# supabase/etl

Hardware: AMD Instinct MI355X
Metric: WAL bytes/s decoded (higher is better)
Workload: dtype u8; 1 GPU; cfg2_fixed_5xint4: 64 MiB batches of CopyData-framed pgoutput, device-resident in / device-resident out, offsets sidecar, NO_CONTROL | ASYNC; batch_bytes=67108819, frames_per_batch=594511, pool_batches=6, parallelism=shard1

## Files before the change

etl_amd/csrc/dev_types.h:

```cpp
#pragma once
#include <stdint.h>

namespace etlg {

enum : uint8_t { FT_BAD = 0 };

struct DevCol {
  uint8_t cls;
  uint8_t nullable;
  uint8_t identity;
  uint8_t key_col;
  uint16_t off_full;
  uint16_t off_key;
  uint16_t key_index;
  uint16_t hr;
};

struct DevSlot {
  uint32_t n_cols, n_ident;
  uint32_t row_full, row_key;
  uint32_t st_full, st_key;
  uint32_t cols_base;
  uint32_t has_var;
  uint32_t key_masks;
// ... 130 lines not shown
  uint32_t keys_base;
};

struct PlanParams {
  unsigned long long* desc;
  unsigned long long* d_clear;
  uint32_t clear_words;
  uint32_t ntiles;
  uint32_t lds_bytes;
  uint32_t rows_off;
  uint32_t n_tabs;
  const PlanTab* tabs;
  const uint32_t* cols;
  uint32_t dbg;
  uint32_t max_row_dw;
  const unsigned long long* pre;
  unsigned long long* pre_out;
  uint32_t* pre_ticket;
  uint32_t pre_tag;
  uint32_t pre_row_dw;
  uint32_t pre_key_dw;
  uint32_t pre_key_below;
  uint32_t pre_key_max;
};

struct ColSel {
  const uint8_t* ev_kind; const uint8_t* ev_flags; const uint32_t* ev_slot; const uint64_t* ev_body;
  uint64_t n_events;
  uint32_t slot, kinds;
  unsigned long long* host_rows;
  uint32_t row_full, row_key;
  uint32_t* blk;
  uint32_t nblocks;
  uint64_t* row_event; uint64_t* row_base;
  uint32_t pb, n_cols;
  uint32_t identity_pk;
  uint32_t pk_comparable;
  const uint8_t* fixed; const uint8_t* heap;
  const uint32_t* cols;
  const uint32_t* kcols;
  uint32_t dl, dl_ident;
  unsigned long long* ice;
};
constexpr unsigned long long kPbDelete = 1ull << 63, kPbKey = 1ull << 62, kPbSecond = 1ull << 61, kPbBase = (1ull << 61) - 1;

constexpr uint32_t kAkNumericStr = 64, kAkTimetzStr = 65, kAkJsonStr = 66;
// ... 74 lines not shown
```

etl_amd/csrc/host_orchestrate.inc:

```

namespace {

int32_t download_batch(etlg_ctx* c, etlg_batch* b) {
  OutSet* os = b->dev;
  if (!os) return ETLG_OK;
  if (!c->d2h_stream) HIPCHK(c, hipStreamCreateWithFlags(&c->d2h_stream, hipStreamNonBlocking));
  hipStream_t s = c->d2h_stream;
  etlg_batch_view& v = b->v;
  const size_t n = (size_t)v.n_events;
  const size_t o_start = 0, o_commit = o_start + al64(n * 8), o_ord = o_commit + al64(n * 8), o_body = o_ord + al64(n * 8);
  const size_t o_table = o_body + al64(n * 8), o_slot = o_table + al64(n * 4), o_kind = o_slot + al64(n * 4), o_flags = o_kind + al64(n);
  const size_t o_fixed = o_flags + al64(n), o_heap = o_fixed + al64((size_t)v.fixed_bytes), total = o_heap + al64((size_t)v.heap_bytes) + 64;
  if (b->h_arena_cap < total) {
    if (b->h_arena) { c->harena_pool.emplace_back(b->h_arena, b->h_arena_cap); b->h_arena = nullptr; b->h_arena_cap = 0; }
    size_t best = (size_t)-1;
    for (size_t i = 0; i < c->harena_pool.size(); i++)
      if (c->harena_pool[i].second >= total && (best == (size_t)-1 || c->harena_pool[i].second < c->harena_pool[best].second)) best = i;
    if (best != (size_t)-1) {
      b->h_arena = c->harena_pool[best].first; b->h_arena_cap = c->harena_pool[best].second;
      c->harena_pool.erase(c->harena_pool.begin() + (long)best);
    } else {
      const size_t cap = (total + (total >> 2) + 4095) & ~(size_t)4095;
      HIPCHK(c, hipHostMalloc((void**)&b->h_arena, cap, hipHostMallocDefault));
      b->h_arena_cap = cap;
// ... 314 lines not shown
  const uint64_t nf_avg = b->scan_chained && b->nf_est ? b->nf_est : nf;
  const uint64_t avg = (b->len + nf_avg - 1) / nf_avg;
  if (level == 0) {
    PlanParams& q = c->pq;
    q.ntiles = (nf + 63) / 64;
    uint64_t cap = 64 * avg * (100 + (uint64_t)c->plan_margin_pct) / 100 + 128;
    cap = std::min<uint64_t>((cap + 127) & ~127ull, 48 * 1024);
    q.rows_off = (uint32_t)std::max<uint64_t>(cap, 2048 + 64);
    q.lds_bytes = q.rows_off + (c->plan_max_row > 32 ? (uint32_t)(64ull * c->plan_max_row + 64) : 0u);
    q.n_tabs = c->n_plan_tabs; q.tabs = (const PlanTab*)((const uint8_t*)b->side->dev.p + b->side->o_ptabs); q.cols = (const uint32_t*)((const uint8_t*)b->side->dev.p + b->side->o_pcols);
    q.dbg = c->plan_dbg;
    q.max_row_dw = (c->plan_max_row + 3) / 4;
    const size_t gtiles = std::min<size_t>(64, (size_t)1 << etlg_k_plan_pre_group_log());
    const size_t per = 2 * ((size_t)q.ntiles + ((size_t)q.ntiles + gtiles - 1) / gtiles);
    const bool pre = c->plan_pre != 0 && c->plan_uniform_dw != 0;
    const size_t dbytes = per * 8 + 64;
    q.desc = nullptr; q.d_clear = nullptr; q.clear_words = 0;
    if (!pre) {
      uint8_t *dcur, *doth;
      RC(take_descriptors(c, dbytes, &dcur, &doth));
      q.desc = (unsigned long long*)dcur;
      q.d_clear = (unsigned long long*)doth; q.clear_words = (uint32_t)(dbytes / 8);
    }
    q.pre = nullptr; q.pre_out = nullptr; q.pre_ticket = nullptr; q.pre_tag = 0; q.pre_row_dw = c->plan_uniform_dw;
    q.pre_key_dw = c->plan_uniform_key_dw; q.pre_key_below = c->plan_deletes ? c->plan_key_below : 0u; q.pre_key_max = c->plan_deletes ? c->plan_key_max : 0u;
    if (pre) {
      constexpr uint32_t NB = etlg_ctx::kPreBufs;
      const size_t pbytes = (64 + per * 8 + 255) & ~(size_t)255;
      if (pbytes > c->pre_half) {
        HIPCHK(c, sync_decode_streams(c));
        const size_t half = (pbytes * 2 + 4095) & ~(size_t)4095;
        HIPCHK(c, c->d_pre.ensure(half * NB));
        HIPCHK(c, hipMemsetAsync(c->d_pre.p, 0, half * NB, c->stream));
        HIPCHK(c, hipStreamSynchronize(c->stream));
        c->pre_half = half;
      }
      const uint32_t useq = c->pre_seq++, slot = useq % NB;
      uint8_t* pbuf = (uint8_t*)c->d_pre.p + (size_t)slot * c->pre_half;
      q.pre_ticket = (uint32_t*)pbuf;
      q.pre_out = (unsigned long long*)(pbuf + 64);
      q.pre_tag = 1u + (useq / NB) % 3u;
      launch(c, kPlanPre, p);
      q.pre = q.pre_out;
      if (c->plan_pre == 1) q.dbg |= 512u;
    }
    launch(c, kPlan, p);
    b->used_fused = true; b->used_cells = false;
    return ETLG_OK;
  }
  FusedParams& q = c->fq;
  bool any_var = false;
  for (int32_t li : c->last_live) for (auto& sc : c->slots[(size_t)li]->cols) if (!fixed_class(sc.type_class)) any_var = true;
  int kernel = (avg <= 192 && !(any_var && cells_ok && avg > 96)) ? 0 : (cells_ok ? 2 : 1);
  if (c->fused_kernel >= 0 && c->fused_kernel <= 2) kernel = c->fused_kernel == 2 && !cells_ok ? 1 : c->fused_kernel;
  if (direct) kernel = 2;
  b->used_rows = false;
  if (kernel != 0 || c->fused_kernel == 4) {
    uint32_t maxh = 1, maxh_old = 0, maxrow = 16;
    bool ok = !b->copy.active && !(p.flags & kDecCopyRows) && !b->any_sync_done && !(c->fused_dbg & ~(8u | 32u)) && q.side_bytes != 0 && ((uintptr_t)p.in & 15) == 0 &&
              widest <= etlg_k_rows_max_cols() && !b->no_rows && c->rows_mode != 0 && (c->fused_kernel < 0 || c->fused_kernel == 4);
    for (int32_t li : c->last_live) {
      const SlotHost& sh = *c->slots[(size_t)li];
      uint32_t nh = 0, nhi = 0;
      for (auto& sc : sh.cols) if (!heapless_class(sc.type_class)) { nh++; if (sc.identity) nhi++; }
      maxh = std::max(maxh, nh); maxh_old = std::max(maxh_old, nhi);
      maxrow = std::max<uint32_t>(maxrow, sh.desc.row_bytes_full + std::max<uint32_t>(sh.desc.row_bytes_key, sh.desc.n_ident == sh.desc.n_cols ? sh.desc.row_bytes_full : 0u));
    }
// ... 531 lines not shown
```

etl_amd/csrc/host_state.h:

```cpp
#pragma once
#include <hip/hip_runtime_api.h>

#include <algorithm>
#include <cstddef>
#include <cstdio>
#include <cstdlib>
#include <cstring>
#include <chrono>
#include <map>
#include <mutex>
#include <memory>
#include <set>
#include <string>
#include <string_view>
#include <type_traits>
#include <unordered_map>
#include <vector>

#include "../../include/etlg.h"
#include "dev_types.h"

using namespace etlg;

extern "C" void etlg_k_launch(int which, const DecParams* p, hipStream_t s);
extern "C" const char* etlg_k_name(int which);
extern "C" void etlg_k_ctl_pick(const uint8_t* tags, uint32_t nframes, uint32_t* hdr, uint32_t* list, uint32_t cap, hipStream_t s);
extern "C" void etlg_k_shard_cuts(const uint8_t* tags, const uint32_t* offs, uint32_t nframes, uint32_t n_shards, uint32_t* cuts, hipStream_t s);
extern "C" void etlg_k_ctl_span(const uint8_t* tags, uint32_t nframes, const uint32_t* list, uint32_t n, uint32_t* span, hipStream_t s);
extern "C" void etlg_k_ctl_gather(const uint8_t* in, const uint32_t* offs, const uint32_t* frames, uint32_t nkeep, uint32_t* lens, const uint32_t* out_offs, uint8_t* out, hipStream_t s);
extern "C" void etlg_k_launch_fused(int blk, const DecParams* p, const void* q, hipStream_t s);
extern "C" int etlg_k_fused_set_lds(void);
extern "C" void etlg_k_launch_bounds(const uint8_t* in, uint64_t len, uint32_t* offs, uint32_t offs_cap, void* scratch, uint32_t* result, uint32_t* hints, uint32_t* hflag,
                                     int sequential, hipStream_t s);
extern "C" size_t etlg_k_bounds_scratch_bytes(size_t ntiles);
extern "C" uint32_t etlg_k_bounds_tile_bytes(void);
extern "C" uint32_t etlg_k_copy_bytes_per_row(uint32_t ncols);
extern "C" int etlg_k_copy_set_lds(void);
extern "C" void etlg_k_launch_copy(const uint8_t* rows, const uint32_t* row_offs, uint32_t nrows, uint64_t rows_len, uint32_t ncols,
                                   uint32_t rel_id, uint8_t* out, uint32_t* out_offs, uint32_t lds_bytes, int lane_per_byte, const DecParams* dec, hipStream_t s);
extern "C" void etlg_k_launch_cells(const DecParams* p, const void* q, hipStream_t s);
extern "C" void etlg_k_launch_plan(const DecParams* p, const void* q, hipStream_t s);
extern "C" void etlg_k_launch_plan_pre(const DecParams* p, const void* q, hipStream_t s);
extern "C" uint32_t etlg_k_plan_pre_group_log(void);
extern "C" int etlg_k_plan_set_lds(void);
extern "C" void etlg_k_col_select(const void* sel, hipStream_t s);
extern "C" void etlg_k_col_cdc(const void* job, hipStream_t s);
extern "C" void etlg_k_col_fixed(const void* job, hipStream_t s);
extern "C" uint32_t etlg_k_col_pack_max(void);
extern "C" void etlg_k_col_fixed_pack(const void* jobs, uint32_t n, hipStream_t s);
extern "C" void etlg_k_col_var_pack(const void* jobs, uint32_t n, unsigned long long* const* blk, int64_t* const* offs, unsigned long long* const* tot, int step, hipStream_t s);
extern "C" void etlg_k_scan_lens(const uint32_t* lens, uint64_t n, unsigned long long* blk, int64_t* offsets, hipStream_t s);
extern "C" void etlg_k_col_list(const void* job, unsigned long long* blk, int64_t* offsets, int step, hipStream_t s);
extern "C" void etlg_k_size_hints(const void* job, hipStream_t s);
extern "C" void etlg_k_rowbinary(const void* job, unsigned long long* blk, int64_t* offsets, unsigned long long* tot, int step, hipStream_t s);
extern "C" void etlg_k_col_var(const void* job, unsigned long long* blk, int64_t* offsets, int step, hipStream_t s);
extern "C" int etlg_k_cells_set_lds(void);
extern "C" uint32_t etlg_k_cells_table_bytes(uint32_t maxc);
extern "C" uint32_t etlg_k_copy_cells_table_bytes(uint32_t maxc);
extern "C" uint32_t etlg_k_copy_cells_lds(uint32_t maxc, uint32_t window);
extern "C" void etlg_k_launch_copy_cells(const DecParams* p, const void* q, hipStream_t s);
extern "C" uint32_t etlg_k_cells_maxc(void);
extern "C" void etlg_k_launch_rows(const DecParams* p, const void* q, hipStream_t s);
extern "C" void etlg_k_finish(const void* job, unsigned long long* blk, int64_t* offsets, int step, hipStream_t st);
extern "C" int etlg_k_rows_set_lds(void);
extern "C" int etlg_k_rows_waves(void);
extern "C" int etlg_k_rows_waves_per_simd(void);
// ... 205 lines not shown
  int users = 0;
  hipEvent_t ready = nullptr;
  uint32_t synced = 0;
};

}

struct etlg_ctx {
  int device = 0;
  uint64_t gen = 0;
  hipStream_t stream = nullptr;
  bool own_stream = false;
  int32_t worker = ETLG_WORKER_APPLY;
  uint32_t sync_table = 0;
  uint64_t bootstrap = 0;
  ControlState cs;
  std::map<uint32_t, TState> states;
  std::vector<std::unique_ptr<SlotHost>> slots;
  bool slots_dirty = true;
  bool in_txn = false; uint64_t final_lsn = 0, next_ord = 0;
  size_t desc_half = 0;
  static constexpr uint32_t kPreBufs = 4;
  DevBuf d_pre; size_t pre_half = 0; uint32_t pre_seq = 0;
  size_t desc_dirty[4] = {0, 0, 0, 0};
  uint32_t desc_cur = 0;
  hipStream_t stream2 = nullptr;
  hipEvent_t tail2 = nullptr;
  bool tail2_set = false;
  hipEvent_t fence_ev = nullptr;
  bool hdr_in_flight = false;
  int overlap_mode = 1;
  bool debug_invariants = false;
  bool prof_serial = false;
  unsigned long long overlapped = 0;
  static constexpr uint32_t kResRing = 32;
  uint64_t scan_last_nf = 0, scan_last_len = 0;
  bool scan_chain_mode = true;
  uint64_t scan_chained_n = 0, scan_chain_redone = 0;
  bool chain_spare = true;
  uint64_t chain_spared = 0;
  uint64_t chain_healed = 0;
  uint64_t ring_recleared = 0;
  uint32_t res_seq = 0;
  DevResult* h_init_ring = nullptr;
  DevResult* d_init_ring = nullptr;
  CopyJob copy;
// ... 172 lines not shown
```

etl_amd/csrc/plan.hip:

```cpp
#include "lookback.hip.h"

namespace etlg {

struct WinLds {
  const ETLG_LDS_AS u8* base;
  DEV uint32_t w(uint32_t aoff) const { return ETLG_LDS_LD32(base + aoff); }
};
struct WinGlb {
  const u8* base; uint32_t lim;
  DEV uint32_t w(uint32_t aoff) const {
    uint32_t v = 0;
    if (aoff + 4 <= lim) __builtin_memcpy(&v, base + aoff, 4);
    else for (uint32_t k = 0; aoff + k < lim; k++) v |= (uint32_t)base[aoff + k] << (8 * k);
    return v;
  }
};
template <class M> DEV uint32_t rd32(const M& m, uint32_t off) {
  const uint32_t a = off & ~3u, s = off & 3u;
  return __builtin_amdgcn_alignbyte(m.w(a + 4), m.w(a), s);
}
template <class M> DEV uint64_t rd64(const M& m, uint32_t off) {
  const uint32_t a = off & ~3u, s = off & 3u;
  const uint32_t w0 = m.w(a), w1 = m.w(a + 4), w2 = m.w(a + 8);
  return __builtin_amdgcn_alignbyte(w1, w0, s) | ((uint64_t)__builtin_amdgcn_alignbyte(w2, w1, s) << 32);
// ... 41 lines not shown
    const uint32_t d2 = dig4(pad_word(__builtin_amdgcn_alignbyte(w3, w2, s), k, 2), bad);
    mag = (uint64_t)d0 * 100000000ull + (d1 * 10000u + d2);
    uint64_t lim;
    if (cls == ETLG_TC_U32) lim = 0xFFFFFFFFull;
    else if (cls == ETLG_TC_I16) lim = neg ? 0x8000ull : 0x7FFFull;
    else lim = neg ? 0x80000000ull : 0x7FFFFFFFull;
    ok = (n != 0u) & (nd != 0u) & (n <= 12u) & (nd <= 11u) & (bad == 0u) & (mag <= lim) & ((cls != ETLG_TC_U32) | (neg ^ 1u));
  }
  return neg ? 0 - mag : mag;
}

DEV int plan_find(const PlanParams& q, uint32_t rel_u) {
  const ETLG_CONST_AS uint32_t* t = (const ETLG_CONST_AS uint32_t*)(uintptr_t)q.tabs;
  int lo = 0, hi = (int)q.n_tabs - 1;
  while (lo <= hi) {
    const int mid = (lo + hi) >> 1;
    const uint32_t v = t[mid * (int)(sizeof(PlanTab) / 4)];
    if (v == rel_u) return mid;
    if (v < rel_u) lo = mid + 1; else hi = mid - 1;
  }
  return -1;
}

#define WSTAMP(k) do { if ((q.dbg & 64u) && threadIdx.x == 0) ((unsigned long long*)p.heap)[(size_t)blockIdx.x * 8 + (k)] = wall_clock64(); } while (0)
#define PSTAMP(k) do { if ((q.dbg & 32u) && threadIdx.x == 0 && (blockIdx.x & 15u) == 3u) { const unsigned long long t_ = clock64(); atomicAdd(&p.res->dbg_t[k], t_ - tprev); tprev = t_; } } while (0)

constexpr uint32_t kPreBeginLen = kBodyOff + 20u, kPreCommitLen = kBodyOff + 25u;
constexpr int kPreTilesPerWave = 8, kPreWaves = 8;
constexpr uint32_t pre_log2(uint32_t v) { return v <= 1u ? 0u : 1u + pre_log2(v >> 1); }
constexpr uint32_t kPreGroupLog = pre_log2(kPreTilesPerWave * kPreWaves);
static_assert((1u << kPreGroupLog) == (uint32_t)(kPreTilesPerWave * kPreWaves), "a group of the pre-pass is a power of two of tiles");
static_assert(kPreTilesPerWave <= 32 && kPreWaves <= 8, "cand_m / short_m are 32-bit masks; at most two waves per SIMD");
constexpr uint32_t kPlanMaxPolls = 1u << 15;

struct PlanPre2 { unsigned long long a0 = 0, l0 = 0, a1 = 0, l1 = 0; bool valid = false; };
struct PlanFold { uint32_t fx, mk, l0, l1; };
DEV PlanFold fold_id() { return PlanFold{0u, 0u, 0u, 0u}; }
DEV PlanFold fold_f(const PlanFold& a, const PlanFold& b) {
  return PlanFold{a.fx + b.fx, a.mk > b.mk ? a.mk : b.mk, b.mk ? b.l0 : a.l0, b.mk ? b.l1 : a.l1};
}
DEV PlanFold fold_of(unsigned long long a, unsigned long long l) {
  return PlanFold{(uint32_t)a, (uint32_t)(a >> 32) & 0x3FFFFFFFu, (uint32_t)l, (uint32_t)(l >> 32) & 0x3FFFFFFFu};
}
DEV unsigned long long fold_agg(const PlanFold& v) { return ((unsigned long long)v.mk << 32) | v.fx; }
DEV unsigned long long fold_lsn(const PlanFold& v) { return ((unsigned long long)v.l1 << 32) | v.l0; }
DEV unsigned long long pair_state(unsigned long long a, unsigned long long l) { const unsigned long long st = a & ST_MASK; return st == (l & ST_MASK) ? st : 0ull; }
DEV PlanFold fold_scan(PlanFold v) {
#define ETLG_P3_DPP(ctrl, rmask) { PlanFold o_; \
    o_.fx = (uint32_t)__builtin_amdgcn_update_dpp(0, (int)v.fx, ctrl, rmask, 0xF, false); o_.mk = (uint32_t)__builtin_amdgcn_update_dpp(0, (int)v.mk, ctrl, rmask, 0xF, false); \
    o_.l0 = (uint32_t)__builtin_amdgcn_update_dpp(0, (int)v.l0, ctrl, rmask, 0xF, false); o_.l1 = (uint32_t)__builtin_amdgcn_update_dpp(0, (int)v.l1, ctrl, rmask, 0xF, false); \
    v = fold_f(o_, v); }
  ETLG_P3_DPP(0x111, 0xF) ETLG_P3_DPP(0x112, 0xF) ETLG_P3_DPP(0x114, 0xF) ETLG_P3_DPP(0x118, 0xF) ETLG_P3_DPP(0x142, 0xA) ETLG_P3_DPP(0x143, 0xC)
#undef ETLG_P3_DPP
  return v;
}
// ... 280 lines not shown
  if (keep) {
#pragma unroll
    for (int d = 0; d < RD; d++) L.row[d] = rimg[d];
  }
  L.agg = agg; L.tile_lsn = tile_lsn; L.ex = ex; L.ex_lsn = ex_lsn; L.tot_mark = tot_mark; L.tot_fx = tot_fx; L.early = early; L.done = false;
}

DEV void plan_late_carry(DecParams& p, uint32_t* failp) {
  if (!(p.flags & 16u) || !p.carry) return;
  for (uint32_t polls = 0;; polls++) {
    if (__hip_atomic_load(&p.carry->carry_ready, __ATOMIC_ACQUIRE, __HIP_MEMORY_SCOPE_AGENT)) break;
    if (polls > kPlanMaxPolls) { if (threadIdx.x == 0) atomicOr(failp, 1u); break; }
    __builtin_amdgcn_s_sleep(8);
  }
  p.in_txn = __hip_atomic_load(&p.carry->out_in_txn, __ATOMIC_RELAXED, __HIP_MEMORY_SCOPE_AGENT);
  p.final_lsn = __hip_atomic_load(&p.carry->out_final_lsn, __ATOMIC_RELAXED, __HIP_MEMORY_SCOPE_AGENT);
  p.next_ord = __hip_atomic_load(&p.carry->out_next_ord, __ATOMIC_RELAXED, __HIP_MEMORY_SCOPE_AGENT);
  p.flags &= ~16u;
}

struct PlanPreWords { unsigned long long g0 = 0, g1 = 0, t0 = 0, t1 = 0; };
DEV PlanPreWords plan_pre_load(const PlanParams& q, uint32_t tile) {
  PlanPreWords w;
  if (q.pre && tile < q.ntiles) {
    const ETLG_CONST_AS unsigned long long* dt = (const ETLG_CONST_AS unsigned long long*)(uintptr_t)(q.pre + 2 * (size_t)tile);
    const ETLG_CONST_AS unsigned long long* dg = (const ETLG_CONST_AS unsigned long long*)(uintptr_t)(q.pre + 2 * ((size_t)q.ntiles + (tile >> kPreGroupLog)));
    w.t0 = dt[0]; w.t1 = dt[1]; w.g0 = dg[0]; w.g1 = dg[1];
  }
  return w;
}

template <int RD>
DEV void plan_resolve(DecParams& p, const PlanParams& q, uint32_t tile, PlanLocal<RD>& L, unsigned long long& tprev, const PlanPre2& pre = PlanPre2(), const PlanPreWords& pw = PlanPreWords()) {
  if (L.done) return;
  const uint32_t lane = threadIdx.x;
  const uint32_t f = tile * 64u + lane;
  uint32_t* failp = &p.res->fused_fail;
  uint32_t bad = L.bad;
  const bool isI = (L.tagf >> 16) & 1u, isB = (L.tagf >> 17) & 1u, isC = (L.tagf >> 18) & 1u;
  const uint32_t pm = L.pm;
  const uint64_t b_lsn = L.b_lsn;
  uint64_t ex = L.ex, ex_lsn = L.ex_lsn;

  if (q.pre) {
    const PlanFold r = fold_f(fold_of(pw.g0, pw.g1), fold_of(pw.t0, pw.t1));
    ex = fold_agg(r); ex_lsn = fold_lsn(r);
  }
  else if (!L.early) plan_resolve2(q.desc, q.desc + 2 * (size_t)q.ntiles, tile, L.agg, L.tile_lsn, failp, pre, ex, ex_lsn);
  PSTAMP(7);
  uint32_t pre_mark = (uint32_t)(ex >> 32);
  if (pre_mark == 0) {
    plan_late_carry(p, failp);
    if (p.in_txn) { pre_mark = 1u; ex |= 1ull << 32; }
  }
  const uint64_t pre_lsn = (pre_mark & 1u) && (pre_mark >> 1) != 0 ? ex_lsn : p.final_lsn;
  PSTAMP(4);
  WSTAMP(4);

  const uint32_t last = pre_mark > pm ? pre_mark : pm;
  const bool in_txn = (last & 1u) != 0;
  const uint32_t fb1 = last >> 1;
  uint64_t final_lsn = 0;
  {
    const bool here = in_txn && fb1 != 0 && fb1 - 1 >= tile * 64u;
    const uint32_t src = here ? fb1 - 1 - tile * 64u : 0u;
    const uint32_t lo = (uint32_t)__shfl((int)(uint32_t)b_lsn, (int)src, 64), hi = (uint32_t)__shfl((int)(uint32_t)(b_lsn >> 32), (int)src, 64);
    if (in_txn) final_lsn = here ? (((uint64_t)hi << 32) | lo) : pre_lsn;
  }
// ... 69 lines not shown
    const uint32_t payu = wave_last(wave_scan_add(is_upd ? vbytes : 0u));
    if (lane == 0 && payu) atomicAdd(&p.res->pay_shard[tile & 31][1], (unsigned long long)payu);
  }
  if (__ballot(is_del && vbytes != 0)) {
    const uint32_t payd = wave_last(wave_scan_add(is_del ? vbytes : 0u));
    if (lane == 0 && payd) atomicAdd(&p.res->pay_shard[tile & 31][2], (unsigned long long)payd);
  }
  if ((any_bad || !cap_ok) && lane == 0) atomicOr(failp, 2u);
}

struct TileSpan { uint32_t nt, span0, span1, my_o; };
DEV TileSpan plan_span(const DecParams& p, uint32_t tile) {
  const uint32_t lane = threadIdx.x;
  TileSpan t;
  const uint32_t f0 = tile * 64u;
  t.nt = p.nframes - f0 < 64u ? p.nframes - f0 : 64u;
  const ETLG_CONST_AS uint32_t* offs_c = (const ETLG_CONST_AS uint32_t*)(uintptr_t)p.offs;
  t.span0 = offs_c[f0]; t.span1 = offs_c[f0 + t.nt];
  t.my_o = lane < t.nt ? p.offs[f0 + lane] : t.span1;
  return t;
}

template <int RD>
DEV void plan_stage_local(DecParams& p, const PlanParams& q, u8* smem, uint32_t tile, const TileSpan& ts, unsigned long long& tprev, PlanLocal<RD>& L, bool keep) {
  const uint32_t lane = threadIdx.x;
  L.done = true;
  const uint32_t nt = ts.nt, span0 = ts.span0, span1 = ts.span1, my_o = ts.my_o;
  PSTAMP(0);
  const uint32_t a0 = span0 & ~15u;
  const bool staged = span1 > span0 && span1 <= p.in_len && (uint64_t)(span1 - a0) + 64 <= q.rows_off && !(q.dbg & 1u);
  if (staged) {
    const uint32_t npieces = (span1 - a0 + 1023u) >> 10;
    for (uint32_t k = 0; k < npieces; k++) {
      const uint32_t c = a0 + (k << 10) + (lane << 4);
      if (c < span1 && (uint64_t)c + 16 <= p.in_len) ETLG_GLDS16(p.in + c, smem + (k << 10));
    }
    const uint32_t tail = a0 + (((uint32_t)p.in_len - a0) & ~15u);
    if (tail < span1 && (uint64_t)tail + 16 > p.in_len && tail + lane < p.in_len && lane < 16) smem[tail - a0 + lane] = p.in[tail + lane];
    ETLG_VMEM_WAIT();
    PSTAMP(1);
    WSTAMP(1);
    if (q.dbg & 2u) { if (smem[lane * 97u] == 0xEE && smem[lane * 13u + 5u] == 0xEF && my_o == 0xFFFFFFF1u) atomicOr(&p.res->fused_fail, 2u); return; }
    const WinLds m{(const ETLG_LDS_AS u8*)smem};
    plan_local(p, q, m, smem, true, a0, tile, nt, my_o, span0, span1, tprev, L, keep);
  } else {
    const WinGlb m{p.in, (uint32_t)p.in_len};
    plan_local(p, q, m, smem, false, 0u, tile, nt, my_o, span0, span1, tprev, L, keep);
  }
}

DEV bool plan_frames_from_device(DecParams& p, PlanParams& q) {
  if (!p.nframes_dev) return true;
  const ETLG_CONST_AS uint32_t* r = (const ETLG_CONST_AS uint32_t*)(uintptr_t)p.nframes_dev;
  const uint32_t nf = r[0], flags = r[1] | r[2];
  if (flags != 0 || nf == 0 || nf > p.nframes) {
    if (blockIdx.x == 0 && threadIdx.x == 0) {
      atomicOr(&p.res->fused_fail, 32u);
      __hip_atomic_store(&p.res->carry_ready, 1u, __ATOMIC_RELEASE, __HIP_MEMORY_SCOPE_AGENT);
    }
    return false;
  }
  p.nframes = nf;
  q.ntiles = (nf + 63u) >> 6;
  return true;
}

template <bool TWO, int RD>
DEV void plan_kernel(DecParams& p, const PlanParams& q_in, u8* smem) {
  PlanParams q = q_in;
  const uint32_t lane = threadIdx.x;
  unsigned long long tprev = (q.dbg & 32u) ? clock64() : 0ull;
  const uint32_t tile = blockIdx.x;
  WSTAMP(0);
  if (q.clear_words) {
    const uint32_t per = (q.clear_words + gridDim.x - 1) / gridDim.x;
    for (uint32_t i = lane; i < per; i += 64) { const uint32_t w = blockIdx.x * per + i; if (w < q.clear_words) q.d_clear[w] = 0; }
  }
  if (!(p.flags & 16u) && !load_carry(p)) return;
  if (!plan_frames_from_device(p, q)) return;
  const uint32_t t0 = TWO ? 2u * blockIdx.x : blockIdx.x;
  if (t0 >= q.ntiles) return;
  const TileSpan sa = plan_span(p, t0);
  const PlanPreWords pwa = plan_pre_load(q, t0), pwb = TWO ? plan_pre_load(q, t0 + 1u) : PlanPreWords();
  TileSpan sb = sa;
  if (TWO && t0 + 1u < q.ntiles) sb = plan_span(p, t0 + 1u);
  PlanLocal<RD> A;
  plan_stage_local(p, q, smem, t0, sa, tprev, A, TWO);
  if (TWO) {
    const uint32_t t1 = t0 + 1u;
    PlanLocal<RD> B;
    B.done = true;
    if (t1 < q.ntiles) {
      __threadfence_block();
      __syncthreads();
      plan_stage_local(p, q, smem, t1, sb, tprev, B, false);
    }
    PlanPre2 preA, preB;
    if (!A.done && !A.early && !q.pre) preA = plan_prefetch2(q.desc, q.desc + 2 * (size_t)q.ntiles, t0);
    if (!B.done && !B.early && !q.pre) preB = plan_prefetch2(q.desc, q.desc + 2 * (size_t)q.ntiles, t1);
    plan_resolve(p, q, t0, A, tprev, preA, pwa);
    plan_resolve(p, q, t1, B, tprev, preB, pwb);
    plan_store<true>(p, q, t0, A, tprev);
    plan_store<false>(p, q, t1, B, tprev);
  } else {
    plan_resolve(p, q, t0, A, tprev, PlanPre2(), pwa);
    plan_store<false>(p, q, t0, A, tprev);
  }
}

__global__ __launch_bounds__(kPreWaves * 64) void k_plan_pre(DecParams p, PlanParams q) {
  __shared__ unsigned long long s_wagg[kPreWaves][2];
  if (!plan_frames_from_device(p, q)) return;
  if (blockIdx.x >= ((q.ntiles + (1u << kPreGroupLog) - 1u) >> kPreGroupLog)) return;
  const uint32_t lane = threadIdx.x & 63u, wave = (uint32_t)__builtin_amdgcn_readfirstlane((int)(threadIdx.x >> 6)), g = blockIdx.x;
  const uint32_t t0 = (g << kPreGroupLog) + wave * (uint32_t)kPreTilesPerWave;
  uint32_t o[kPreTilesPerWave + 1];
#pragma unroll
  for (int i = 0; i <= kPreTilesPerWave; i++) {
    const uint64_t f = (uint64_t)(t0 + (uint32_t)i) * 64u + lane;
    o[i] = p.offs[f < p.nframes ? f : p.nframes];
  }
  uint32_t cand_m = 0;
  uint32_t short_m = 0;
  uint32_t tagv[kPreTilesPerWave];
  uint64_t lsnv[kPreTilesPerWave];
#pragma unroll
  for (int i = 0; i < kPreTilesPerWave; i++) {
    const uint64_t f = (uint64_t)(t0 + (uint32_t)i) * 64u + lane;
    const uint32_t o0 = o[i];
    const uint32_t nxt = (uint32_t)__builtin_amdgcn_readfirstlane((int)o[i + 1]);
    const uint32_t o1 = (uint32_t)__builtin_amdgcn_update_dpp((int)nxt, (int)o0, 0x130, 0xF, 0xF, false);
    const uint32_t flen = o1 - o0;
    const bool cand = f < p.nframes && o1 > o0 && o1 <= p.in_len && (flen == kPreBeginLen || flen == kPreCommitLen || (flen >= q.pre_key_below && flen <= q.pre_key_max));
    tagv[i] = 0; lsnv[i] = 0;
    if (cand) { cand_m |= 1u << i; tagv[i] = p.in[o0 + 30] | (flen << 8); lsnv[i] = ld_be64(p.in + o0 + 31); }
    if (flen < q.pre_key_below) short_m |= 1u << i;
  }
  PlanFold run = fold_id();
  PlanFold keep = fold_id();
#pragma unroll
  for (int i = 0; i < kPreTilesPerWave; i++) {
    const uint32_t tile = t0 + (uint32_t)i;
    const uint64_t f = (uint64_t)tile * 64u + lane;
    const bool live = f < p.nframes;
    const bool cand = (cand_m >> i) & 1u;
    const uint32_t tag = tagv[i] & 0xFFu, flen = tagv[i] >> 8;
    const uint64_t lsn = lsnv[i];
    const bool isB = cand && flen == kPreBeginLen && tag == 'B', isC = cand && flen == kPreCommitLen && tag == 'C';
    const bool isDel = ((short_m >> i) & 1u) || (cand && tag == 'D' && flen <= q.pre_key_max);
    const unsigned long long mB = __ballot(isB), mC = __ballot(isC), mD = __ballot(live && isDel && !isB && !isC);
    const uint64_t base = (uint64_t)tile * 64u;
    const uint32_t nlive = base >= p.nframes ? 0u : (p.nframes - base < 64u ? (uint32_t)(p.nframes - base) : 64u);
    const uint32_t nB = (uint32_t)__builtin_popcountll(mB), nC = (uint32_t)__builtin_popcountll(mC), nD = (uint32_t)__builtin_popcountll(mD);
    const uint32_t tot_fx = 2u * nB + 4u * nC + q.pre_key_dw * nD + q.pre_row_dw * (nlive - nB - nC - nD);
    const unsigned long long mBC = mB | mC;
    uint32_t tot_mark = 0;
    if (mBC) {
      const uint32_t h = 63u - (uint32_t)__builtin_clzll(mBC);
      tot_mark = ((((uint32_t)base + h) + 1u) << 1) | (uint32_t)((mB >> h) & 1ull);
    }
    uint64_t tile_lsn = 0;
    if (tot_mark & 1u) {
      const int src = (int)((tot_mark >> 1) - 1u - tile * 64u);
      tile_lsn = ((uint64_t)(uint32_t)__builtin_amdgcn_readlane((int)(uint32_t)(lsn >> 32), src) << 32) | (uint32_t)__builtin_amdgcn_readlane((int)(uint32_t)lsn, src);
      tile_lsn &= ~(3ull << 62);
    }
    if (lane == (uint32_t)i) keep = run;
    run = fold_f(run, PlanFold{tot_fx, tot_mark, (uint32_t)tile_lsn, (uint32_t)(tile_lsn >> 32)});
  }
  if (lane == 0) { s_wagg[wave][0] = fold_agg(run); s_wagg[wave][1] = fold_lsn(run); }
  __syncthreads();
  PlanFold before = fold_id();
  for (uint32_t w = 0; w < wave; w++) before = fold_f(before, fold_of(s_wagg[w][0], s_wagg[w][1]));
  if (lane < (uint32_t)kPreTilesPerWave && t0 + lane < q.ntiles) {
    const PlanFold r = fold_f(before, keep);
    unsigned long long* d = q.pre_out + 2 * (size_t)(t0 + lane);
    d[0] = fold_agg(r); d[1] = fold_lsn(r);
  }
  if (wave != (uint32_t)kPreWaves - 1u) return;
  const uint32_t ng = (q.ntiles + (1u << kPreGroupLog) - 1u) >> kPreGroupLog;
  unsigned long long* gd = q.pre_out + 2 * (size_t)q.ntiles;
  const unsigned long long tagbits = (unsigned long long)q.pre_tag << 62;
  uint32_t ticket = 0;
  if (lane == 0) {
    const PlanFold all = fold_f(before, run);
    ETLG_ST_PAIR(gd + 2 * (size_t)g, tagbits | fold_agg(all), tagbits | fold_lsn(all));
    ticket = atomicAdd(q.pre_ticket, 1u);
  }
  ticket = (uint32_t)__builtin_amdgcn_readfirstlane((int)ticket);
  if (ticket != ng - 1u) return;
  PlanFold carry = fold_id();
  unsigned long long na = 0, nl = 0;
// ... 1 lines not shown
  for (uint32_t base = 0; base < ng; base += 64u) {
    const uint32_t gi = base + lane;
    unsigned long long a = gi < ng ? na : tagbits, l = gi < ng ? nl : tagbits;
    if (gi + 64u < ng) ETLG_LD_PAIR(gd + 2 * (size_t)(gi + 64u), na, nl);
    bool have = pair_state(a, l) == tagbits;
    bool gave_up = false;
    for (uint32_t polls = 0;; polls++) {
      if (!have) { ETLG_LD_PAIR(gd + 2 * (size_t)gi, a, l); have = pair_state(a, l) == tagbits; }
      if (!__ballot(!have)) break;
      if (polls > kPlanMaxPolls) { if (lane == 0) atomicOr(&p.res->fused_fail, 1u); gave_up = true; break; }
      __builtin_amdgcn_s_sleep(2);
    }
    const PlanFold inc = fold_scan(gi < ng ? fold_of(a, l) : fold_id());
    PlanFold exc;
    exc.fx = (uint32_t)__builtin_amdgcn_update_dpp(0, (int)inc.fx, 0x138, 0xF, 0xF, false); exc.mk = (uint32_t)__builtin_amdgcn_update_dpp(0, (int)inc.mk, 0x138, 0xF, 0xF, false);
    exc.l0 = (uint32_t)__builtin_amdgcn_update_dpp(0, (int)inc.l0, 0x138, 0xF, 0xF, false); exc.l1 = (uint32_t)__builtin_amdgcn_update_dpp(0, (int)inc.l1, 0x138, 0xF, 0xF, false);
    const PlanFold r = fold_f(carry, exc);
    if (gi < ng && !gave_up) { gd[2 * (size_t)gi] = fold_agg(r); gd[2 * (size_t)gi + 1] = fold_lsn(r); }
    carry = fold_f(carry, fold_lane63(inc));
  }
  if (lane == 0) __hip_atomic_store(q.pre_ticket, 0u, __ATOMIC_RELAXED, __HIP_MEMORY_SCOPE_AGENT);
}

__global__ __launch_bounds__(64, ETLG_PLAN_MINWAVES) void k_plan(DecParams p, PlanParams q) {
  ETLG_DYNAMIC_LDS(smem);
  plan_kernel<false, 1>(p, q, smem);
}

template <int RD>
__global__ __launch_bounds__(64, ETLG_PLAN_MINWAVES) void k_plan2(DecParams p, PlanParams q) {
  ETLG_DYNAMIC_LDS(smem);
  plan_kernel<true, RD>(p, q, smem);
}

}

extern "C" {

using namespace etlg;

void etlg_k_launch_plan_pre(const DecParams* p, const void* qv, hipStream_t s) {
  const PlanParams* q = (const PlanParams*)qv;
  hipLaunchKernelGGL(k_plan_pre, dim3((q->ntiles + (1u << kPreGroupLog) - 1u) >> kPreGroupLog), dim3(kPreWaves * 64), 0, s, *p, *q);
}

void etlg_k_launch_plan(const DecParams* p, const void* qv, hipStream_t s) {
  const PlanParams* q = (const PlanParams*)qv;
  if (q->lds_bytes == q->rows_off && q->max_row_dw <= 8u && !(q->dbg & 512u)) {
    if (q->max_row_dw <= 6u) hipLaunchKernelGGL(k_plan2<6>, dim3((q->ntiles + 1) / 2), dim3(64), q->lds_bytes, s, *p, *q);
    else hipLaunchKernelGGL(k_plan2<8>, dim3((q->ntiles + 1) / 2), dim3(64), q->lds_bytes, s, *p, *q);
  } else hipLaunchKernelGGL(k_plan, dim3(q->ntiles), dim3(64), q->lds_bytes, s, *p, *q);
}

uint32_t etlg_k_plan_pre_group_log(void) { return kPreGroupLog; }

int etlg_k_plan_set_lds(void) {
  const int a = hipFuncSetAttribute((const void*)k_plan, hipFuncAttributeMaxDynamicSharedMemorySize, 64 * 1024) == hipSuccess ? 0 : 1;
  const int b = hipFuncSetAttribute((const void*)k_plan2<6>, hipFuncAttributeMaxDynamicSharedMemorySize, 64 * 1024) == hipSuccess ? 0 : 1;
  const int c = hipFuncSetAttribute((const void*)k_plan2<8>, hipFuncAttributeMaxDynamicSharedMemorySize, 64 * 1024) == hipSuccess ? 0 : 1;
  return a | b | c;
}

}
```

Baseline: 1859 GB/s.

## Fuse plan pre-pass into plan kernel as leading producer and scanner blocks

```diff
diff --git a/etl_amd/csrc/dev_types.h b/etl_amd/csrc/dev_types.h
--- a/etl_amd/csrc/dev_types.h
+++ b/etl_amd/csrc/dev_types.h
@@ -176,6 +176,7 @@
   uint32_t pre_key_dw;
   uint32_t pre_key_below;
   uint32_t pre_key_max;
+  uint32_t pre_fused;
 };
 
 struct ColSel {
diff --git a/etl_amd/csrc/host_orchestrate.inc b/etl_amd/csrc/host_orchestrate.inc
--- a/etl_amd/csrc/host_orchestrate.inc
+++ b/etl_amd/csrc/host_orchestrate.inc
@@ -360,11 +360,16 @@
       q.desc = (unsigned long long*)dcur;
       q.d_clear = (unsigned long long*)doth; q.clear_words = (uint32_t)(dbytes / 8);
     }
-    q.pre = nullptr; q.pre_out = nullptr; q.pre_ticket = nullptr; q.pre_tag = 0; q.pre_row_dw = c->plan_uniform_dw;
+    q.pre = nullptr; q.pre_out = nullptr; q.pre_ticket = nullptr; q.pre_tag = 0; q.pre_fused = 0; q.pre_row_dw = c->plan_uniform_dw;
     q.pre_key_dw = c->plan_uniform_key_dw; q.pre_key_below = c->plan_deletes ? c->plan_key_below : 0u; q.pre_key_max = c->plan_deletes ? c->plan_key_max : 0u;
     if (pre) {
       constexpr uint32_t NB = etlg_ctx::kPreBufs;
-      const size_t pbytes = (64 + per * 8 + 255) & ~(size_t)255;
+      const bool fused = c->plan_pre == 3 && !p.nframes_dev;
+      const size_t tpw = etlg_k_plan_fused_tiles_per_wave();
+      const size_t npre = fused ? ((size_t)q.ntiles + tpw - 1) / tpw : 0;
+      const size_t wpt = etlg_k_plan_fused_waves_per_trip();
+      const size_t pwords = fused ? 2 * ((size_t)q.ntiles + 2 * npre + (npre + wpt - 1) / wpt) : per;
+      const size_t pbytes = (64 + pwords * 8 + 255) & ~(size_t)255;
       if (pbytes > c->pre_half) {
         HIPCHK(c, sync_decode_streams(c));
         const size_t half = (pbytes * 2 + 4095) & ~(size_t)4095;
@@ -372,15 +377,22 @@
         HIPCHK(c, hipMemsetAsync(c->d_pre.p, 0, half * NB, c->stream));
         HIPCHK(c, hipStreamSynchronize(c->stream));
         c->pre_half = half;
+        for (uint32_t& e : c->pre_ext) e = 0;
       }
       const uint32_t useq = c->pre_seq++, slot = useq % NB;
       uint8_t* pbuf = (uint8_t*)c->d_pre.p + (size_t)slot * c->pre_half;
       q.pre_ticket = (uint32_t*)pbuf;
       q.pre_out = (unsigned long long*)(pbuf + 64);
       q.pre_tag = 1u + (useq / NB) % 3u;
-      launch(c, kPlanPre, p);
+      if (c->plan_pre == 3) {
+        const uint32_t ahead = (useq + 2u) % NB;
+        q.d_clear = (unsigned long long*)((uint8_t*)c->d_pre.p + (size_t)ahead * c->pre_half + 64); q.clear_words = c->pre_ext[ahead];
+        c->pre_ext[ahead] = 0; c->pre_ext[slot] = (uint32_t)pwords;
+      }
+      if (fused) q.pre_fused = (uint32_t)npre;
+      else launch(c, kPlanPre, p);
       q.pre = q.pre_out;
-      if (c->plan_pre == 1) q.dbg |= 512u;
+      if (c->plan_pre == 1 || fused) q.dbg |= 512u;
     }
     launch(c, kPlan, p);
     b->used_fused = true; b->used_cells = false;
diff --git a/etl_amd/csrc/host_state.h b/etl_amd/csrc/host_state.h
--- a/etl_amd/csrc/host_state.h
+++ b/etl_amd/csrc/host_state.h
@@ -42,6 +42,8 @@
 extern "C" void etlg_k_launch_plan(const DecParams* p, const void* q, hipStream_t s);
 extern "C" void etlg_k_launch_plan_pre(const DecParams* p, const void* q, hipStream_t s);
 extern "C" uint32_t etlg_k_plan_pre_group_log(void);
+extern "C" uint32_t etlg_k_plan_fused_tiles_per_wave(void);
+extern "C" uint32_t etlg_k_plan_fused_waves_per_trip(void);
 extern "C" int etlg_k_plan_set_lds(void);
 extern "C" void etlg_k_col_select(const void* sel, hipStream_t s);
 extern "C" void etlg_k_col_cdc(const void* job, hipStream_t s);
@@ -293,6 +295,7 @@
   size_t desc_half = 0;
   static constexpr uint32_t kPreBufs = 4;
   DevBuf d_pre; size_t pre_half = 0; uint32_t pre_seq = 0;
+  uint32_t pre_ext[kPreBufs] = {};
   size_t desc_dirty[4] = {0, 0, 0, 0};
   uint32_t desc_cur = 0;
   hipStream_t stream2 = nullptr;
diff --git a/etl_amd/csrc/plan.hip b/etl_amd/csrc/plan.hip
--- a/etl_amd/csrc/plan.hip
+++ b/etl_amd/csrc/plan.hip
@@ -87,8 +87,10 @@
   return -1;
 }
 
-#define WSTAMP(k) do { if ((q.dbg & 64u) && threadIdx.x == 0) ((unsigned long long*)p.heap)[(size_t)blockIdx.x * 8 + (k)] = wall_clock64(); } while (0)
-#define PSTAMP(k) do { if ((q.dbg & 32u) && threadIdx.x == 0 && (blockIdx.x & 15u) == 3u) { const unsigned long long t_ = clock64(); atomicAdd(&p.res->dbg_t[k], t_ - tprev); tprev = t_; } } while (0)
+DEV uint32_t plan_fused_groups(uint32_t np) { return (np + 63u) >> 6; }
+DEV uint32_t plan_fused_front(const PlanParams& q) { return q.pre_fused + plan_fused_groups(q.pre_fused); }
+#define WSTAMP(k) do { if ((q.dbg & 64u) && threadIdx.x == 0) ((unsigned long long*)p.heap)[(size_t)(blockIdx.x - plan_fused_front(q)) * 8 + (k)] = wall_clock64(); } while (0)
+#define PSTAMP(k) do { if ((q.dbg & 32u) && threadIdx.x == 0 && ((blockIdx.x - plan_fused_front(q)) & 15u) == 3u) { const unsigned long long t_ = clock64(); atomicAdd(&p.res->dbg_t[k], t_ - tprev); tprev = t_; } } while (0)
 
 constexpr uint32_t kPreBeginLen = kBodyOff + 20u, kPreCommitLen = kBodyOff + 25u;
 constexpr int kPreTilesPerWave = 8, kPreWaves = 8;
@@ -96,6 +98,9 @@
 constexpr uint32_t kPreGroupLog = pre_log2(kPreTilesPerWave * kPreWaves);
 static_assert((1u << kPreGroupLog) == (uint32_t)(kPreTilesPerWave * kPreWaves), "a group of the pre-pass is a power of two of tiles");
 static_assert(kPreTilesPerWave <= 32 && kPreWaves <= 8, "cand_m / short_m are 32-bit masks; at most two waves per SIMD");
+constexpr int kFusedTilesPerWave = 8;
+constexpr uint32_t kFusedWavesPerTrip = 64;
+static_assert(kFusedWavesPerTrip == 64u, "a group scanner takes one pre-wave per lane");
 constexpr uint32_t kPlanMaxPolls = 1u << 15;
 
 struct PlanPre2 { unsigned long long a0 = 0, l0 = 0, a1 = 0, l1 = 0; bool valid = false; };
@@ -422,7 +427,7 @@
 struct PlanPreWords { unsigned long long g0 = 0, g1 = 0, t0 = 0, t1 = 0; };
 DEV PlanPreWords plan_pre_load(const PlanParams& q, uint32_t tile) {
   PlanPreWords w;
-  if (q.pre && tile < q.ntiles) {
+  if (q.pre && !q.pre_fused && tile < q.ntiles) {
     const ETLG_CONST_AS unsigned long long* dt = (const ETLG_CONST_AS unsigned long long*)(uintptr_t)(q.pre + 2 * (size_t)tile);
     const ETLG_CONST_AS unsigned long long* dg = (const ETLG_CONST_AS unsigned long long*)(uintptr_t)(q.pre + 2 * ((size_t)q.ntiles + (tile >> kPreGroupLog)));
     w.t0 = dt[0]; w.t1 = dt[1]; w.g0 = dg[0]; w.g1 = dg[1];
@@ -430,8 +435,56 @@
   return w;
 }
 
+struct PlanFusedWords { unsigned long long t0 = 0, t1 = 0, w0 = 0, w1 = 0; uint32_t packed = 0; };
+DEV const unsigned long long* plan_fused_tile_word(const PlanParams& q, uint32_t tile) { return q.pre + 2 * (size_t)tile; }
+DEV const unsigned long long* plan_fused_wave_word(const PlanParams& q, uint32_t tile) {
+  return q.pre + 2 * ((size_t)q.ntiles + q.pre_fused + tile / (uint32_t)kFusedTilesPerWave);
+}
+DEV unsigned long long plan_uniform64(unsigned long long v) {
+  return ((unsigned long long)(uint32_t)__builtin_amdgcn_readfirstlane((int)(uint32_t)(v >> 32)) << 32) | (uint32_t)__builtin_amdgcn_readfirstlane((int)(uint32_t)v);
+}
+DEV PlanFusedWords plan_fused_request(const PlanParams& q, uint32_t tile) {
+  PlanFusedWords f;
+  if (q.pre_fused && tile < q.ntiles) {
+    ETLG_LD_PAIR(plan_fused_tile_word(q, tile), f.t0, f.t1);
+    ETLG_LD_PAIR(plan_fused_wave_word(q, tile), f.w0, f.w1);
+  }
+  return f;
+}
+DEV void plan_fused_settle(const PlanParams& q, PlanFusedWords& f) {
+  const unsigned long long tagbits = (unsigned long long)q.pre_tag << 62;
+  const unsigned long long t0 = plan_uniform64(f.t0), t1 = plan_uniform64(f.t1), w0 = plan_uniform64(f.w0), w1 = plan_uniform64(f.w1);
+  const uint32_t have = (pair_state(t0, t1) == tagbits && pair_state(w0, w1) == tagbits) ? 1u : 0u;
+  const PlanFold r = fold_f(fold_of(w0, w1), fold_of(t0, t1));
+  const uint32_t lane = threadIdx.x;
+  f.packed = lane == 0 ? r.fx : lane == 1 ? r.mk : lane == 2 ? r.l0 : lane == 3 ? r.l1 : have;
+  f.t0 = f.t1 = f.w0 = f.w1 = 0;
+}
+DEV PlanFold plan_fused_resolve(const PlanParams& q, uint32_t tile, const PlanFusedWords& f, uint32_t* failp) {
+  if (__builtin_amdgcn_readlane((int)f.packed, 4))
+    return PlanFold{(uint32_t)__builtin_amdgcn_readlane((int)f.packed, 0), (uint32_t)__builtin_amdgcn_readlane((int)f.packed, 1),
+                    (uint32_t)__builtin_amdgcn_readlane((int)f.packed, 2), (uint32_t)__builtin_amdgcn_readlane((int)f.packed, 3)};
+  const unsigned long long tagbits = (unsigned long long)q.pre_tag << 62;
+  PlanFold r = fold_id();
+  uint32_t polls = 0;
+  for (int k = 0; k < 2; k++) {
+    const unsigned long long* src = k == 0 ? plan_fused_wave_word(q, tile) : plan_fused_tile_word(q, tile);
+    unsigned long long a, l;
+    for (;; polls++) {
+      ETLG_LD_PAIR(src, a, l);
+      a = plan_uniform64(a); l = plan_uniform64(l);
+      if (pair_state(a, l) == tagbits) break;
+      if (polls > kPlanMaxPolls) { if (threadIdx.x == 0) atomicOr(failp, 1u); return fold_id(); }
+      __builtin_amdgcn_s_sleep(2);
+    }
+    r = fold_f(r, fold_of(a, l));
+  }
+  return r;
+}
+
 template <int RD>
-DEV void plan_resolve(DecParams& p, const PlanParams& q, uint32_t tile, PlanLocal<RD>& L, unsigned long long& tprev, const PlanPre2& pre = PlanPre2(), const PlanPreWords& pw = PlanPreWords()) {
+DEV void plan_resolve(DecParams& p, const PlanParams& q, uint32_t tile, PlanLocal<RD>& L, unsigned long long& tprev, const PlanPre2& pre = PlanPre2(), const PlanPreWords& pw = PlanPreWords(),
+                      const PlanFusedWords& fw = PlanFusedWords()) {
   if (L.done) return;
   const uint32_t lane = threadIdx.x;
   const uint32_t f = tile * 64u + lane;
@@ -443,7 +496,7 @@
   uint64_t ex = L.ex, ex_lsn = L.ex_lsn;
 
   if (q.pre) {
-    const PlanFold r = fold_f(fold_of(pw.g0, pw.g1), fold_of(pw.t0, pw.t1));
+    const PlanFold r = q.pre_fused ? plan_fused_resolve(q, tile, fw, failp) : fold_f(fold_of(pw.g0, pw.g1), fold_of(pw.t0, pw.t1));
     ex = fold_agg(r); ex_lsn = fold_lsn(r);
   }
   else if (!L.early) plan_resolve2(q.desc, q.desc + 2 * (size_t)q.ntiles, tile, L.agg, L.tile_lsn, failp, pre, ex, ex_lsn);
@@ -559,7 +612,7 @@
 }
 
 template <int RD>
-DEV void plan_stage_local(DecParams& p, const PlanParams& q, u8* smem, uint32_t tile, const TileSpan& ts, unsigned long long& tprev, PlanLocal<RD>& L, bool keep) {
+DEV void plan_stage_local(DecParams& p, const PlanParams& q, u8* smem, uint32_t tile, const TileSpan& ts, unsigned long long& tprev, PlanLocal<RD>& L, bool keep, PlanFusedWords& fw) {
   const uint32_t lane = threadIdx.x;
   L.done = true;
   const uint32_t nt = ts.nt, span0 = ts.span0, span1 = ts.span1, my_o = ts.my_o;
@@ -574,13 +627,16 @@
     }
     const uint32_t tail = a0 + (((uint32_t)p.in_len - a0) & ~15u);
     if (tail < span1 && (uint64_t)tail + 16 > p.in_len && tail + lane < p.in_len && lane < 16) smem[tail - a0 + lane] = p.in[tail + lane];
+    if (q.pre_fused) fw = plan_fused_request(q, tile);
     ETLG_VMEM_WAIT();
+    if (q.pre_fused) plan_fused_settle(q, fw);
     PSTAMP(1);
     WSTAMP(1);
     if (q.dbg & 2u) { if (smem[lane * 97u] == 0xEE && smem[lane * 13u + 5u] == 0xEF && my_o == 0xFFFFFFF1u) atomicOr(&p.res->fused_fail, 2u); return; }
     const WinLds m{(const ETLG_LDS_AS u8*)smem};
     plan_local(p, q, m, smem, true, a0, tile, nt, my_o, span0, span1, tprev, L, keep);
   } else {
+    if (q.pre_fused) { fw = plan_fused_request(q, tile); plan_fused_settle(q, fw); }
     const WinGlb m{p.in, (uint32_t)p.in_len};
     plan_local(p, q, m, smem, false, 0u, tile, nt, my_o, span0, span1, tprev, L, keep);
   }
@@ -602,27 +658,32 @@
   return true;
 }
 
+DEV void plan_fused_pre_wave(DecParams& p, const PlanParams& q);
+DEV void plan_fused_scanner(DecParams& p, const PlanParams& q);
+
 template <bool TWO, int RD>
 DEV void plan_kernel(DecParams& p, const PlanParams& q_in, u8* smem) {
   PlanParams q = q_in;
   const uint32_t lane = threadIdx.x;
   unsigned long long tprev = (q.dbg & 32u) ? clock64() : 0ull;
-  const uint32_t tile = blockIdx.x;
-  WSTAMP(0);
   if (q.clear_words) {
     const uint32_t per = (q.clear_words + gridDim.x - 1) / gridDim.x;
     for (uint32_t i = lane; i < per; i += 64) { const uint32_t w = blockIdx.x * per + i; if (w < q.clear_words) q.d_clear[w] = 0; }
   }
+  const uint32_t nfront = TWO ? 0u : q.pre_fused + plan_fused_groups(q.pre_fused);
+  if (blockIdx.x < nfront) { if (blockIdx.x < q.pre_fused) plan_fused_pre_wave(p, q); else plan_fused_scanner(p, q); return; }
+  WSTAMP(0);
   if (!(p.flags & 16u) && !load_carry(p)) return;
   if (!plan_frames_from_device(p, q)) return;
-  const uint32_t t0 = TWO ? 2u * blockIdx.x : blockIdx.x;
+  const uint32_t t0 = TWO ? 2u * blockIdx.x : blockIdx.x - nfront;
   if (t0 >= q.ntiles) return;
   const TileSpan sa = plan_span(p, t0);
   const PlanPreWords pwa = plan_pre_load(q, t0), pwb = TWO ? plan_pre_load(q, t0 + 1u) : PlanPreWords();
+  PlanFusedWords fwa;
   TileSpan sb = sa;
   if (TWO && t0 + 1u < q.ntiles) sb = plan_span(p, t0 + 1u);
   PlanLocal<RD> A;
-  plan_stage_local(p, q, smem, t0, sa, tprev, A, TWO);
+  plan_stage_local(p, q, smem, t0, sa, tprev, A, TWO, fwa);
   if (TWO) {
     const uint32_t t1 = t0 + 1u;
     PlanLocal<RD> B;
@@ -630,7 +691,7 @@
     if (t1 < q.ntiles) {
       __threadfence_block();
       __syncthreads();
-      plan_stage_local(p, q, smem, t1, sb, tprev, B, false);
+      plan_stage_local(p, q, smem, t1, sb, tprev, B, false, fwa);
     }
     PlanPre2 preA, preB;
     if (!A.done && !A.early && !q.pre) preA = plan_prefetch2(q.desc, q.desc + 2 * (size_t)q.ntiles, t0);
@@ -640,29 +701,25 @@
     plan_store<true>(p, q, t0, A, tprev);
     plan_store<false>(p, q, t1, B, tprev);
   } else {
-    plan_resolve(p, q, t0, A, tprev, PlanPre2(), pwa);
+    plan_resolve(p, q, t0, A, tprev, PlanPre2(), pwa, fwa);
     plan_store<false>(p, q, t0, A, tprev);
   }
 }
 
-__global__ __launch_bounds__(kPreWaves * 64) void k_plan_pre(DecParams p, PlanParams q) {
-  __shared__ unsigned long long s_wagg[kPreWaves][2];
-  if (!plan_frames_from_device(p, q)) return;
-  if (blockIdx.x >= ((q.ntiles + (1u << kPreGroupLog) - 1u) >> kPreGroupLog)) return;
-  const uint32_t lane = threadIdx.x & 63u, wave = (uint32_t)__builtin_amdgcn_readfirstlane((int)(threadIdx.x >> 6)), g = blockIdx.x;
-  const uint32_t t0 = (g << kPreGroupLog) + wave * (uint32_t)kPreTilesPerWave;
-  uint32_t o[kPreTilesPerWave + 1];
+template <int T>
+DEV void plan_pre_wave_fold(const DecParams& p, const PlanParams& q, uint32_t t0, uint32_t lane, PlanFold& run, PlanFold& keep) {
+  uint32_t o[T + 1];
 #pragma unroll
-  for (int i = 0; i <= kPreTilesPerWave; i++) {
+  for (int i = 0; i <= T; i++) {
     const uint64_t f = (uint64_t)(t0 + (uint32_t)i) * 64u + lane;
     o[i] = p.offs[f < p.nframes ? f : p.nframes];
   }
   uint32_t cand_m = 0;
   uint32_t short_m = 0;
-  uint32_t tagv[kPreTilesPerWave];
-  uint64_t lsnv[kPreTilesPerWave];
+  uint32_t tagv[T];
+  uint64_t lsnv[T];
 #pragma unroll
-  for (int i = 0; i < kPreTilesPerWave; i++) {
+  for (int i = 0; i < T; i++) {
     const uint64_t f = (uint64_t)(t0 + (uint32_t)i) * 64u + lane;
     const uint32_t o0 = o[i];
     const uint32_t nxt = (uint32_t)__builtin_amdgcn_readfirstlane((int)o[i + 1]);
@@ -673,10 +730,10 @@
     if (cand) { cand_m |= 1u << i; tagv[i] = p.in[o0 + 30] | (flen << 8); lsnv[i] = ld_be64(p.in + o0 + 31); }
     if (flen < q.pre_key_below) short_m |= 1u << i;
   }
-  PlanFold run = fold_id();
-  PlanFold keep = fold_id();
+  run = fold_id();
+  keep = fold_id();
 #pragma unroll
-  for (int i = 0; i < kPreTilesPerWave; i++) {
+  for (int i = 0; i < T; i++) {
     const uint32_t tile = t0 + (uint32_t)i;
     const uint64_t f = (uint64_t)tile * 64u + lane;
     const bool live = f < p.nframes;
@@ -705,6 +762,16 @@
     if (lane == (uint32_t)i) keep = run;
     run = fold_f(run, PlanFold{tot_fx, tot_mark, (uint32_t)tile_lsn, (uint32_t)(tile_lsn >> 32)});
   }
+}
+
+__global__ __launch_bounds__(kPreWaves * 64) void k_plan_pre(DecParams p, PlanParams q) {
+  __shared__ unsigned long long s_wagg[kPreWaves][2];
+  if (!plan_frames_from_device(p, q)) return;
+  if (blockIdx.x >= ((q.ntiles + (1u << kPreGroupLog) - 1u) >> kPreGroupLog)) return;
+  const uint32_t lane = threadIdx.x & 63u, wave = (uint32_t)__builtin_amdgcn_readfirstlane((int)(threadIdx.x >> 6)), g = blockIdx.x;
+  const uint32_t t0 = (g << kPreGroupLog) + wave * (uint32_t)kPreTilesPerWave;
+  PlanFold run, keep;
+  plan_pre_wave_fold<kPreTilesPerWave>(p, q, t0, lane, run, keep);
   if (lane == 0) { s_wagg[wave][0] = fold_agg(run); s_wagg[wave][1] = fold_lsn(run); }
   __syncthreads();
   PlanFold before = fold_id();
@@ -752,7 +819,58 @@
   if (lane == 0) __hip_atomic_store(q.pre_ticket, 0u, __ATOMIC_RELAXED, __HIP_MEMORY_SCOPE_AGENT);
 }
 
-__global__ __launch_bounds__(64, ETLG_PLAN_MINWAVES) void k_plan(DecParams p, PlanParams q) {
+#define PWSTAMP(k) do { if ((q.dbg & 64u) && threadIdx.x == 0 && ((size_t)q.ntiles + blockIdx.x + 1) * 64 <= p.heap_cap) ((unsigned long long*)p.heap)[((size_t)q.ntiles + blockIdx.x) * 8 + (k)] = wall_clock64(); } while (0)
+DEV void plan_fused_pre_wave(DecParams& p, const PlanParams& q) {
+  const uint32_t lane = threadIdx.x, w = blockIdx.x;
+  const uint32_t t0 = w * (uint32_t)kFusedTilesPerWave;
+  PWSTAMP(0);
+  PlanFold run, keep;
+  plan_pre_wave_fold<kFusedTilesPerWave>(p, q, t0, lane, run, keep);
+  const unsigned long long tagbits = (unsigned long long)q.pre_tag << 62;
+  if (lane < (uint32_t)kFusedTilesPerWave && t0 + lane < q.ntiles) ETLG_ST_PAIR(q.pre_out + 2 * (size_t)(t0 + lane), tagbits | fold_agg(keep), tagbits | fold_lsn(keep));
+  if (lane == 0) ETLG_ST_PAIR(q.pre_out + 2 * ((size_t)q.ntiles + w), tagbits | fold_agg(run), tagbits | fold_lsn(run));
+  PWSTAMP(1);
+}
+DEV bool plan_fused_poll_scan(const DecParams& p, const unsigned long long* src, uint32_t first, uint32_t n, unsigned long long tagbits, PlanFold& inc) {
+  const uint32_t lane = threadIdx.x;
+  unsigned long long a = tagbits, l = tagbits;
+  bool have = lane >= n;
+  for (uint32_t polls = 0;; polls++) {
+    if (!have) { ETLG_LD_PAIR(src + 2 * (size_t)(first + lane), a, l); have = pair_state(a, l) == tagbits; }
+    if (!__ballot(!have)) break;
+    if (polls > kPlanMaxPolls) { if (lane == 0) atomicOr(&p.res->fused_fail, 1u); return false; }
+    __builtin_amdgcn_s_sleep(2);
+  }
+  inc = fold_scan(lane < n ? fold_of(a, l) : fold_id());
+  return true;
+}
+DEV void plan_fused_scanner(DecParams& p, const PlanParams& q) {
+  const uint32_t lane = threadIdx.x, np = q.pre_fused, g = blockIdx.x - np;
+  const unsigned long long tagbits = (unsigned long long)q.pre_tag << 62;
+  unsigned long long* wagg = q.pre_out + 2 * (size_t)q.ntiles;
+  unsigned long long* wex = wagg + 2 * (size_t)np;
+  unsigned long long* gagg = wex + 2 * (size_t)np;
+  const uint32_t w0 = g * kFusedWavesPerTrip, n = np - w0 < kFusedWavesPerTrip ? np - w0 : kFusedWavesPerTrip;
+  PWSTAMP(0);
+  PlanFold inc;
+  if (!plan_fused_poll_scan(p, wagg, w0, n, tagbits, inc)) return;
+  const PlanFold all = fold_lane63(inc);
+  if (lane == 0) ETLG_ST_PAIR(gagg + 2 * (size_t)g, tagbits | fold_agg(all), tagbits | fold_lsn(all));
+  PlanFold exc;
+  exc.fx = (uint32_t)__builtin_amdgcn_update_dpp(0, (int)inc.fx, 0x138, 0xF, 0xF, false); exc.mk = (uint32_t)__builtin_amdgcn_update_dpp(0, (int)inc.mk, 0x138, 0xF, 0xF, false);
+  exc.l0 = (uint32_t)__builtin_amdgcn_update_dpp(0, (int)inc.l0, 0x138, 0xF, 0xF, false); exc.l1 = (uint32_t)__builtin_amdgcn_update_dpp(0, (int)inc.l1, 0x138, 0xF, 0xF, false);
+  PlanFold before = fold_id();
+  for (uint32_t base = 0; base < g; base += 64u) {
+    PlanFold ginc;
+    if (!plan_fused_poll_scan(p, gagg, base, g - base < 64u ? g - base : 64u, tagbits, ginc)) return;
+    before = fold_f(before, fold_lane63(ginc));
+  }
+  const PlanFold r = fold_f(before, exc);
+  if (lane < n) ETLG_ST_PAIR(wex + 2 * (size_t)(w0 + lane), tagbits | fold_agg(r), tagbits | fold_lsn(r));
+  PWSTAMP(1);
+}
+
+__global__ __launch_bounds__(64, ETLG_PLAN_MINWAVES + 1) void k_plan(DecParams p, PlanParams q) {
   ETLG_DYNAMIC_LDS(smem);
   plan_kernel<false, 1>(p, q, smem);
 }
@@ -776,12 +894,15 @@
 
 void etlg_k_launch_plan(const DecParams* p, const void* qv, hipStream_t s) {
   const PlanParams* q = (const PlanParams*)qv;
-  if (q->lds_bytes == q->rows_off && q->max_row_dw <= 8u && !(q->dbg & 512u)) {
+  if (q->pre_fused) hipLaunchKernelGGL(k_plan, dim3(q->pre_fused + (q->pre_fused + kFusedWavesPerTrip - 1) / kFusedWavesPerTrip + q->ntiles), dim3(64), q->lds_bytes, s, *p, *q);
+  else if (q->lds_bytes == q->rows_off && q->max_row_dw <= 8u && !(q->dbg & 512u)) {
     if (q->max_row_dw <= 6u) hipLaunchKernelGGL(k_plan2<6>, dim3((q->ntiles + 1) / 2), dim3(64), q->lds_bytes, s, *p, *q);
     else hipLaunchKernelGGL(k_plan2<8>, dim3((q->ntiles + 1) / 2), dim3(64), q->lds_bytes, s, *p, *q);
   } else hipLaunchKernelGGL(k_plan, dim3(q->ntiles), dim3(64), q->lds_bytes, s, *p, *q);
 }
 
+uint32_t etlg_k_plan_fused_tiles_per_wave(void) { return (uint32_t)kFusedTilesPerWave; }
+uint32_t etlg_k_plan_fused_waves_per_trip(void) { return kFusedWavesPerTrip; }
 uint32_t etlg_k_plan_pre_group_log(void) { return kPreGroupLog; }
 
 int etlg_k_plan_set_lds(void) {
```

After: 1815 GB/s. 2.4% lower.
